# ufukpage/TripleD-Exploring-Depth-Estimation-with-Self-Supervised-Representation-Learning

Hardware: AMD Instinct MI355X
Metric: train imgs/sec at KITTI 192x640 bs=12/GPU (higher is better)
Workload: dtype bf16 convs (MFMA) + f32 loss kernels

## Files before the change

include/tripled_hip.h:

```cpp
#ifndef TRIPLED_HIP_H
#define TRIPLED_HIP_H

#include <stddef.h>
#include <stdint.h>

#ifdef __cplusplus
extern "C" {
#endif

#define TD_ABI_VERSION 3
#define TD_MAX_SRC 4

#define TD_OK 0
#define TD_ERR_BAD_ARG (-1)
#define TD_ERR_UNSUPPORTED (-2)
#define TD_ERR_LAUNCH (-3)
#define TD_ERR_WORKSPACE (-4)

typedef void* td_stream_t;

int td_abi_version(void);
const char* td_error_string(int code);
const char* td_last_hip_error(void);

// ... 90 lines not shown
                     float* workspace, td_stream_t stream);
long long td_conv1x1_wgrad_workspace_floats(long long M, int K, int N);
int td_conv1x1_wgrad(const void* dy, const void* x, long long M, int K, int N, int Hi, int Wi, int stride, int dw_dtype, void* dw,
                     float* workspace, td_stream_t stream);
int td_conv1x1_wgrad_group(int n, const void* const* dy, const void* const* x, const long long* M, const int* K, const int* N,
                           const int* Hi, const int* Wi, const int* stride, const int* dw_dtype, void* const* dw,
                           float* const* workspace, td_stream_t stream);
int td_bn_fwd_from_partials(const void* x, const void* residual, int dtype, const float* gamma, const float* beta,
                            float* running_mean, float* running_var, float momentum, float eps, int relu, long long M,
                            int groups, int C, float* partials, int stat_rows, void* y, float* save_mean,
                            float* save_invstd, td_stream_t stream);

long long td_bias_act_workspace_floats(long long M, int C);
int td_bias_act_fwd(const void* y, const void* bias, int bias_dtype, int dtype, long long M, int C, int act, void* a, td_stream_t stream);
int td_bias_act_bwd(const void* g, const void* a, int dtype, long long M, int C, int act, void* gy, void* dbias, int dbias_dtype,
                    float* workspace, td_stream_t stream);

int td_adam_flat(float* w, const float* grad, float* exp_avg, float* exp_avg_sq, void* lowp, long long n, long long n_lowp,
                 const float* step, const float* lr_dev, float lr_host, double beta1, double beta2, float eps, const float* total_norm,
                 float max_norm, td_stream_t stream);

int td_gather_flat(const void* const* srcs, const long long* dst_offsets, const long long* numels, int n, int src_dtype, float* flat,
                   td_stream_t stream);

int td_bn_partial_rows(long long M, int groups, int C);
int td_bn_fwd_partials(const void* x, int dtype, long long M, int groups, int C, float* partials, td_stream_t stream);
int td_bn_bwd_partials(const void* dy, const void* x, const void* y, int dtype, const float* gamma, const float* beta,
                       const float* save_mean, const float* save_invstd, int relu, long long M, int groups, int C, float* partials,
                       td_stream_t stream);
int td_bn_bwd_from_partials(const void* dy, const void* x, const void* y, int dtype, const float* gamma, const float* beta,
                            const float* save_mean, const float* save_invstd, int relu, long long M, int groups, int C,
                            float* partials, int stat_rows, void* dx, void* dresidual, float* dgamma, float* dbeta,
                            td_stream_t stream);
int td_conv1x1_fwd_bnrelu(const void* z, const void* w, long long M, int groups, int K, int N, float* in_partials, int in_rows,
                          const float* gamma, const float* beta, float* running_mean, float* running_var, float momentum, float eps,
                          float* save_mean, float* save_invstd, void* a_side, void* y, float* stat_partials, td_stream_t stream);
int td_conv1x1_dgrad(const void* dy, const void* w, long long M, int groups, int Cout, int Cin, const void* residual, void* dx,
                     td_stream_t stream);
int td_conv1x1_fwd_sum(const void* x, const void* w, long long M, int K, int N, const void* run_in, void* y, void* run_out,
                       td_stream_t stream);
int td_conv1x1_dgrad_bnsums(const void* dy, const void* w, long long M, int groups, int Cout, int Cin, const void* z,
                            const float* gamma, const float* beta, const float* save_mean, const float* save_invstd, void* dx,
                            float* out_partials, td_stream_t stream);
int td_conv1x1_dgrad_bnbwd(const void* g, const void* z, const void* w, long long M, int groups, int Cout, int Cin, float* in_partials,
                           int in_rows, const float* gamma, const float* beta, const float* save_mean, const float* save_invstd,
                           float* dgamma, float* dbeta, void* dz_side, const void* residual, void* dx, td_stream_t stream);

int td_bn_sync_fwd_sums(const void* x, int dtype, long long M, int groups, int C, float* sums, float* workspace,
                        td_stream_t stream);
int td_bn_sync_fwd_apply(const void* x, const void* residual, int dtype, const float* sums, const float* count,
                         const float* gamma, const float* beta, float* running_mean, float* running_var, float momentum,
                         float eps, int relu, long long M, int groups, int C, void* y, float* save_mean,
                         float* save_invstd, td_stream_t stream);
int td_bn_sync_bwd_sums(const void* dy, const void* x, const void* y, int dtype, const float* gamma, const float* beta,
                        const float* save_mean, const float* save_invstd, int relu, long long M, int groups, int C,
                        float* sums, float* workspace, td_stream_t stream);
int td_bn_sync_bwd_dx(const void* dy, const void* x, const void* y, int dtype, const float* local_sums,
                      const float* global_sums, const float* count, const float* gamma, const float* beta,
                      const float* save_mean, const float* save_invstd, int relu, long long M, int groups, int C,
                      void* dx, void* dresidual, float* dgamma, float* dbeta, float* coef, td_stream_t stream);

int td_edge_weights(const float* img, int B, int h, int w, float a, const float* scale6, float* Wt,
                    td_stream_t stream);
int td_featreg_num_blocks(int B, int h, int w, int C);
int td_featreg_fwd(const void* feat, int dtype, const float* Wt, int B, int h, int w, int C,
                   float* partial, td_stream_t stream);
int td_featreg_bwd(const void* feat, int dtype, const float* Wt, const float* gscale, int B, int h, int w,
                   int C, void* grad, td_stream_t stream);

int td_recon_num_tasks(int B, int h, int w);
int td_recon_fwd(const float* x, const float* y, const float* hole, int B, int h, int w,
                 float* partial, td_stream_t stream);
int td_recon_bwd(const float* x, const float* y, const float* hole, const float* gscale, int B, int h,
                 int w, float* dx, td_stream_t stream);

int td_reflpad1_fwd(const void* in, int dtype, int N, int H, int W, int C, void* out, td_stream_t stream);
int td_reflpad1_bwd(const void* grad_out, int dtype, int N, int H, int W, int C, void* grad_in,
                    td_stream_t stream);

int td_up2_reflpad1_fwd(const void* in, int dtype, int N, int H, int W, int C, void* out, td_stream_t stream);
int td_up2_reflpad1_bwd(const void* grad_out, int dtype, int N, int H, int W, int C, void* grad_in,
                        td_stream_t stream);

int td_featwarp_num_blocks(int B, int h, int w);
int td_featwarp_fwd(const void* tgt, const void* const* src, int n_src, int dtype, const float* disp,
                    const float* P, const float* invK, int B, int h, int w, int C, int hs, int ws,
                    float min_depth, float max_depth, uint8_t* argmin, float* partial, td_stream_t stream);
int td_featwarp_bwd(const void* tgt, const void* const* src, int n_src, int dtype, const float* disp,
                    const float* P, const float* invK, const uint8_t* argmin, const float* gscale,
                    float inv_count, int B, int h, int w, int C, int hs, int ws, float min_depth,
                    float max_depth, void* d_tgt, int* const* d_src, float* d_up, float* dP_partial,
                    td_stream_t stream);
int td_featwarp_dsrc_finish(const int* acc, const float* gscale, float inv_count, int C, long long n, int dtype, void* out,
                            td_stream_t stream);
int td_reduce_partials(const float* partial, int n_src, int B, int blocks_per_sample, float* dP,
                       td_stream_t stream);

int td_l1map_fwd(const void* pred, int dtype, const long long* pred_strides, const float* target, int B, int C,
                 int H, int W, float weight, float* out, td_stream_t stream);
int td_l1map_bwd(const void* pred, int dtype, const long long* pred_strides, const float* target,
                 const float* gmap, int B, int C, int H, int W, float weight, void* dpred, td_stream_t stream);

int td_rgb2lab(const float* rgb, int B, int H, int W, float l_cent, float l_norm, float ab_norm, float* lab,
               td_stream_t stream);

int td_pose_fwd(const float* axisangle, const float* translation, const int* invert, const float* K,
                int n_pairs, int B, float* T, float* P, td_stream_t stream);
int td_pose_bwd(const float* axisangle, const float* translation, const int* invert, const float* K,
                int n_pairs, int B, const float* gT, const float* gP, float* g_axisangle,
                float* g_translation, td_stream_t stream);

int td_color_jitter(const uint8_t* frames_u8, const float* aug, int N, int H, int W, float* means_scratch, float* color,
                    float* color_aug, td_stream_t stream);

int td_fp8_num_blocks(long long n);
int td_fp8_amax_partials(const void* x, int dtype, long long n, float* partials, td_stream_t stream);
int td_fp8_quantize(const void* x, int dtype, long long n, const float* partials, uint8_t* q, float* inv_scale,
                    td_stream_t stream);

#ifdef __cplusplus
}
#endif
#endif
```

tripled-exploring-depth-estimation-with-self-supervised-representation-learning_amd/hostside/mono/model/networks.py:

```python
import os

import numpy as np
import torch
import torch.nn as nn
import torch.nn.functional as F



FUSED_BN_OFF = bool(os.environ.get("TD_NO_FUSED_BN"))


def _ops():
    from tripled_amd import ops
    return ops


def _dense_cl(x):
    if x.is_cuda and x.dim() == 4 and x.shape[1] % 8 == 0 and x.dtype in (torch.float32, torch.bfloat16) \
            and not x.is_contiguous(memory_format=torch.channels_last) and x.stride(1) == 1:
        return x.contiguous(memory_format=torch.channels_last)
    return x


def _fell_back(site, x, why=""):
# ... 451 lines not shown
        self.features = []

    def forward(self, input_image, input_features=None):
        self.features = self.encoder.pyramid(input_image, input_features)
        return self.features

    def stem_only(self, input_image):
        return self.encoder.stem(input_image)


class PoseDecoder(nn.Module):

    def __init__(self, num_ch_enc, stride=1):
        super().__init__()
        self.reduce = Conv2d(int(num_ch_enc[-1]), 256, 1)
        self.conv1 = nn.Conv2d(256, 256, 3, stride, 1)
        self.conv2 = nn.Conv2d(256, 256, 3, stride, 1)
        self.conv3 = nn.Conv2d(256, 6, 1)
        self.relu = nn.ReLU()

    def forward(self, input_features):
        x = self.relu(self.reduce(input_features[-1]))
        x = self.relu(self.conv1(x))
        x = self.relu(self.conv2(x))
        x = self.conv3(x).float()
        x = 0.01 * x.mean(3).mean(2).view(-1, 1, 1, 6)
        return x[..., :3], x[..., 3:]



def upsample(x):
    if x.is_cuda and torch.is_autocast_enabled():
        with torch.autocast("cuda", enabled=False):
            return F.interpolate(x, scale_factor=2, mode="nearest")
    return F.interpolate(x, scale_factor=2, mode="nearest")


class Conv1x1(nn.Module):
    def __init__(self, in_channels, out_channels, bias=False):
        super().__init__()
        self.conv = Conv2d(int(in_channels), int(out_channels), kernel_size=1, stride=1, bias=bias)

    def forward(self, x):
        return self.conv(x)


def _round8(n):
    return (n + 7) // 8 * 8


class _ConvImmediate(torch.autograd.Function):

    @staticmethod
    def forward(ctx, x, w, b):
        with torch.backends.cudnn.flags(enabled=True, benchmark=False):
            y = F.conv2d(x, w, b)
        ctx.save_for_backward(x, w)
        ctx.has_bias = b is not None
        return y

    @staticmethod
    def backward(ctx, gy):
        x, w = ctx.saved_tensors
        with torch.backends.cudnn.flags(enabled=True, benchmark=False):
            gx, gw, gb = torch.ops.aten.convolution_backward(gy, x, w, [w.shape[0]] if ctx.has_bias else None, [1, 1], [0, 0], [1, 1],
                                                              False, [0, 0], 1, [True, True, ctx.has_bias])
        return gx, gw, (gb if ctx.has_bias else None)


class _KeepChannels(torch.autograd.Function):

    @staticmethod
    def forward(ctx, y, c):
        ctx.pad = y.shape[1] - c
        return y.narrow(1, 0, c)

    @staticmethod
    def backward(ctx, g):
        return F.pad(g, (0, 0, 0, 0, 0, ctx.pad)), None


FUSED_BIAS_ACT_OFF = bool(os.environ.get("TD_NO_FUSED_BIAS_ACT"))
FUSED_CRP_OFF = bool(os.environ.get("TD_NO_FUSED_CRP"))


def _activate(y, act):
    if act == "elu":
        return F.elu(y, inplace=True)
    if act == "leaky_relu":
        return F.leaky_relu(y)
    return y


def _conv2d_guarded(x, w, b, act=None):
    if x.is_cuda and x.shape[1] <= 16 and w.shape[0] <= 16 and x.shape[3] > 1024 and torch.backends.cudnn.benchmark:
        if torch.is_autocast_enabled():
            dt = torch.get_autocast_dtype("cuda")
            x, w, b = x.to(dt), w.to(dt), (b.to(dt) if b is not None else None)
        return _activate(_ConvImmediate.apply(x, w, b), act)
    if (act is not None or b is not None) and x.is_cuda and not FUSED_BIAS_ACT_OFF and torch.is_grad_enabled() \
            and torch.is_autocast_enabled() and torch.get_autocast_dtype("cuda") == torch.bfloat16:
        xb = x if x.dtype == torch.bfloat16 else x.to(torch.bfloat16)
        wb = w if w.dtype == torch.bfloat16 else w.to(torch.bfloat16)
        if _ops().conv_bias_act_supported(xb, wb, b, act):
            return _ops().conv_bias_act(xb, wb, b, act)
    return _activate(F.conv2d(x, w, b), act)


class Conv3x3(nn.Module):

    def __init__(self, in_channels, out_channels, use_refl=True):
        super().__init__()
        self.use_refl = use_refl
        self.pad = nn.ReflectionPad2d(1) if use_refl else nn.ZeroPad2d(1)
        self.conv = nn.Conv2d(int(in_channels), int(out_channels), 3)

    def _pad_input(self, x):
        x = _dense_cl(x)
        if self.use_refl and x.shape[1] % 8 == 0 and x.dtype in (torch.float32, torch.bfloat16) \
                and x.is_contiguous(memory_format=torch.channels_last) and x.shape[2] >= 2 and x.shape[3] >= 2:
            from tripled_amd import ops
            return ops.reflpad1(x)
        if self.use_refl:
            _fell_back("Conv3x3.pad", x)
        return self.pad(x)

    def forward(self, x, act=None):
        low_precision = x.is_cuda and (x.dtype == torch.bfloat16 or torch.is_autocast_enabled())
        if not low_precision or os.environ.get("TD_NO_CHANNEL_PAD"):
            return _activate(self.conv(self._pad_input(x) if x.is_cuda else self.pad(x)), act)
        w, b = self.conv.weight, self.conv.bias
        cout, cin = w.shape[0], w.shape[1]
        cin_p, cout_p = _round8(cin), _round8(cout)
        if cin_p == cin and cout_p == cout and x.shape[1] == cin:
            return _conv2d_guarded(self._pad_input(x), w, b, act)
        if x.shape[1] == cin and cin_p != cin:
            x = torch.cat((x, x.new_zeros(x.shape[0], cin_p - cin, x.shape[2], x.shape[3])), 1)
        if x.shape[1] != cin_p:
            raise ValueError("Conv3x3 expects %d (or pre-padded %d) input channels, got %d" % (cin, cin_p, x.shape[1]))
        if not x.is_contiguous(memory_format=torch.channels_last):
            x = x.contiguous(memory_format=torch.channels_last)
        w = F.pad(w, (0, 0, 0, 0, 0, cin_p - cin, 0, cout_p - cout))
        if b is not None and cout_p != cout:
            b = F.pad(b, (0, cout_p - cout))
        if cout_p != cout:
            return _activate(_KeepChannels.apply(_conv2d_guarded(self._pad_input(x), w, b), cout), act)
        return _conv2d_guarded(self._pad_input(x), w, b, act)

    def forward_up(self, x, act=None):
        w, b = self.conv.weight, self.conv.bias
        cout, cin = w.shape[0], w.shape[1]
        x = _dense_cl(x)
        low_precision = x.is_cuda and (x.dtype == torch.bfloat16 or torch.is_autocast_enabled())
        if (self.use_refl and x.is_cuda and x.shape[1] == cin and cin % 8 == 0 and (cout % 8 == 0 or low_precision)
                and x.dtype in (torch.float32, torch.bfloat16) and x.is_contiguous(memory_format=torch.channels_last)
                and not os.environ.get("TD_NO_FUSED_UPSAMPLE")):
            cout_p = _round8(cout)
            if cout_p != cout:
                w = F.pad(w, (0, 0, 0, 0, 0, 0, 0, cout_p - cout))
                b = F.pad(b, (0, cout_p - cout)) if b is not None else None
            if cout_p != cout:
                return _activate(_KeepChannels.apply(_conv2d_guarded(_ops().up2_reflpad1(x), w, b), cout), act)
            return _conv2d_guarded(_ops().up2_reflpad1(x), w, b, act)
        _fell_back("Conv3x3.forward_up", x)
        return self.forward(upsample(x), act)


class Conv5x5(nn.Module):
    def __init__(self, in_channels, out_channels, use_refl=True):
        super().__init__()
        self.pad = nn.ReflectionPad2d(2) if use_refl else nn.ZeroPad2d(2)
        self.conv = nn.Conv2d(int(in_channels), int(out_channels), 5)

    def forward(self, x):
        return self.conv(self.pad(x))


class ConvBlock(nn.Module):
    def __init__(self, in_channels, out_channels):
        super().__init__()
        self.conv = Conv3x3(in_channels, out_channels)
        self.nonlin = nn.ELU(inplace=True)

    def forward(self, x):
        return self.conv(x, act="elu")

    def forward_up(self, x):
        return self.conv.forward_up(x, act="elu")


class CRPBlock(nn.Module):

    def __init__(self, in_planes, out_planes, n_stages):
        super().__init__()
        for i in range(n_stages):
            setattr(self, "{}_{}".format(i + 1, "pointwise"),
                    Conv1x1(in_planes if i == 0 else out_planes, out_planes, False))
        self.stride = 1
        self.n_stages = n_stages
        self.maxpool = nn.MaxPool2d(kernel_size=5, stride=1, padding=2)

    def _pool(self, t):
        if t.is_cuda and t.is_contiguous(memory_format=torch.channels_last) and t.shape[1] % 8 == 0 \
                and t.dtype in (torch.float32, torch.bfloat16):
            from tripled_amd import ops
            return ops.maxpool5(t)
        _fell_back("CRPBlock.maxpool", t)
        return self.maxpool(t)

    def _fused(self, x):
        if FUSED_CRP_OFF or _FP8_1X1[0] or not (self.training and x.is_cuda and torch.is_grad_enabled()):
            return None
        if not (torch.is_autocast_enabled() and torch.get_autocast_dtype("cuda") == torch.bfloat16):
            return None
        convs = [getattr(self, "{}_{}".format(i + 1, "pointwise")).conv for i in range(self.n_stages)]
        if any(c.bias is not None for c in convs):
            return None
        xb = _dense_cl(x if x.dtype == torch.bfloat16 else x.to(torch.bfloat16))
        ws = [c.weight if c.weight.dtype == torch.bfloat16 else c.weight.to(torch.bfloat16) for c in convs]
        if not _ops().crp_supported(xb, ws):
            return None
        return _ops().crp_block(xb, ws)

    def forward(self, x):
        y = self._fused(x)
        if y is not None:
            return y
        top = x
        for i in range(self.n_stages):
            top = getattr(self, "{}_{}".format(i + 1, "pointwise"))(self._pool(top))
            x = top + x
        return x
# ... 37 lines not shown
                setattr(self, "up%d" % i, upshuffle(width, 2))
        self.reduce4 = Conv1x1(num_ch_enc[4], 512, bias=False)
        self.reduce3 = Conv1x1(num_ch_enc[3], width, bias=False)
        self.reduce2 = Conv1x1(num_ch_enc[2], width, bias=False)
        self.reduce1 = Conv1x1(num_ch_enc[1], width, bias=False)
        self.iconv4 = Conv3x3(512, width)
        self.iconv3 = Conv3x3(width * 2 + 1, width)
        self.iconv2 = Conv3x3(width * 2 + 1, width)
        self.iconv1 = Conv3x3(width * 2 + 1, width)
        for i in (4, 3, 2, 1):
            setattr(self, "crp%d" % i, nn.Sequential(CRPBlock(width, width, stages)))
        for i in (4, 3, 2, 1):
            setattr(self, "merge%d" % i, Conv3x3(width, width))
        for i in (4, 3, 2, 1):
            setattr(self, "disp%d" % i, nn.Sequential(Conv3x3(width, 1), nn.Sigmoid()))

    def _stage(self, i, x):
        x = getattr(self, "iconv%d" % i)(x, act="leaky_relu")
        x = getattr(self, "crp%d" % i)(x)
        x = getattr(self, "merge%d" % i)(x, act="leaky_relu")
        head = getattr(self, "disp%d" % i)
        if self.use_shuffle:
            x = getattr(self, "up%d" % (2 if i == 1 else i))(x)
        elif x.is_cuda and x.dtype == torch.bfloat16 and x.is_contiguous(memory_format=torch.channels_last) \
                and x.shape[1] % 8 == 0 and not os.environ.get("TD_NO_FUSED_UPSAMPLE"):
            return x, head[1](head[0].forward_up(x)), True
        else:
            x = upsample(x)
        return x, head(x), False

    def forward(self, input_features, frame_id=0):
        _, l1, l2, l3, l4 = input_features
        l4 = self.do(l4)
        l3 = self.do(l3)
        def joined(r, x, d, deferred):
            if deferred:
                tail = d.to(x.dtype)
                if _ops().join_channels_up2_supported(r, x, tail) and not os.environ.get("TD_NO_CHANNEL_PAD"):
                    return _ops().join_channels_up2(r, x, tail)
                _fell_back("DepthDecoder.join_up2", x)
                x = upsample(x)
            parts = [r, x, d.to(x.dtype)]
            c = sum(p.shape[1] for p in parts)
            if x.is_cuda and c % 8 and x.dtype == torch.bfloat16 and not os.environ.get("TD_NO_CHANNEL_PAD"):
                if _round8(c) == r.shape[1] + x.shape[1] + 8 and _ops().join_channels_supported(*parts):
                    return _ops().join_channels(*parts)
                _fell_back("DepthDecoder.join", x)
                parts.append(x.new_zeros(x.shape[0], _round8(c) - c, x.shape[2], x.shape[3]))
            return torch.cat(parts, 1)

        x, d4, up = self._stage(4, self.reduce4(l4))
        x, d3, up = self._stage(3, joined(self.reduce3(l3), x, d4, up))
        x, d2, up = self._stage(2, joined(self.reduce2(l2), x, d3, up))
        x, d1, up = self._stage(1, joined(self.reduce1(l1), x, d2, up))
        self.outputs = {("disp", frame_id, 3): d4, ("disp", frame_id, 2): d3,
                        ("disp", frame_id, 1): d2, ("disp", frame_id, 0): d1}
        return self.outputs


class Decoder(nn.Module):
    out_key = "res_img"

    def __init__(self, num_ch_enc, num_output_channels=3, num_ch_dec=(16, 32, 64, 128, 256)):
        super().__init__()
        self.num_ch_dec = num_ch_dec
        d = num_ch_dec
        self.upconv5 = ConvBlock(num_ch_enc[4], d[4])
        self.upconv4 = ConvBlock(d[4], d[3])
        self.upconv3 = ConvBlock(d[3], d[2])
        self.upconv2 = ConvBlock(d[2], d[1])
        self.upconv1 = ConvBlock(d[1], d[0])
        self.iconv5 = ConvBlock(d[4], d[4])
        self.iconv4 = ConvBlock(d[3], d[3])
        self.iconv3 = ConvBlock(d[2], d[2])
        self.iconv2 = ConvBlock(d[1], d[1])
        self.iconv1 = ConvBlock(d[0], d[0])
        self.disp4 = Conv3x3(d[3], num_output_channels)
        self.disp3 = Conv3x3(d[2], num_output_channels)
        self.disp2 = Conv3x3(d[1], num_output_channels)
        self.disp1 = Conv3x3(d[0], num_output_channels)
        self.sigmoid = nn.Sigmoid()

    def _heads(self, outputs, key, frame_id, i4, i3, i2, i1):
        outputs[(key, frame_id, 3)] = self.sigmoid(self.disp4(i4))
        outputs[(key, frame_id, 2)] = self.sigmoid(self.disp3(i3))
        outputs[(key, frame_id, 1)] = self.sigmoid(self.disp2(i2))
        outputs[(key, frame_id, 0)] = self.sigmoid(self.disp1(i1))
        return outputs

    def forward(self, input_features, frame_id=0):
        x = self.iconv5.forward_up(self.upconv5(input_features[4]))
        i4 = self.iconv4.forward_up(self.upconv4(x))
        i3 = self.iconv3.forward_up(self.upconv3(i4))
        i2 = self.iconv2.forward_up(self.upconv2(i3))
        i1 = self.iconv1.forward_up(self.upconv1(i2))
        self.outputs = self._heads({}, "res_img", frame_id, i4, i3, i2, i1)
        return self.outputs


class ColorDecoder(Decoder):

    def __init__(self, num_ch_enc, num_output_channels=3, skip_connection_multiplier=1):
        super().__init__(num_ch_enc, num_output_channels, num_ch_dec=(16, 32, 64, 128, 256))
        self.skip_connection_multiplier = skip_connection_multiplier
        d = self.num_ch_dec
        self.upconv5_skip = ConvBlock(num_ch_enc[3], d[3])
        self.upconv4_skip = ConvBlock(num_ch_enc[2], d[2])
        self.upconv3_skip = ConvBlock(num_ch_enc[1], d[1])
        self.upconv2_skip = ConvBlock(num_ch_enc[0], d[0])

    def forward(self, input_features, outputs=None, frame_id=0, skip_layers=(None, None, None, None)):
        e1, e2, e3, e4, e5 = input_features
        m = self.skip_connection_multiplier

        def with_disp(low, scale):
            dsp = F.interpolate(outputs[("disp", frame_id, scale)], [2 * low.shape[2], 2 * low.shape[3]], mode="bilinear",
                                align_corners=False)
            return (dsp * m).to(low.dtype)

        l5 = self.upconv5(e5)
        i5 = self.iconv5.forward_up(l5) + with_disp(l5, 3)
        l4 = self.upconv4(i5)
        if skip_layers[0]:
            l4 = l4 + self.upconv5_skip(e4)
        i4 = self.iconv4.forward_up(l4) + with_disp(l4, 2)
        l3 = self.upconv3(i4)
        if skip_layers[1]:
            l3 = l3 + self.upconv4_skip(e3)
        i3 = self.iconv3.forward_up(l3) + with_disp(l3, 1)
        l2 = self.upconv2(i3)
        if skip_layers[2]:
            l2 = l2 + self.upconv3_skip(e2)
        i2 = self.iconv2.forward_up(l2) + with_disp(l2, 0)
        l1 = self.upconv1(i2)
        if skip_layers[3]:
            l1 = l1 + self.upconv2_skip(e1)
        i1 = self.iconv1.forward_up(l1)
        return self._heads(outputs, "auto_res_img", frame_id, i4, i3, i2, i1)


class IdentityPartial(nn.Module):

    def __init__(self, part_ratio=2, use_right=True):
        super().__init__()
        self.part_ratio = part_ratio
        self.use_right = use_right

    def forward(self, embedding):
        cut = embedding.size(1) // self.part_ratio
        return embedding[:, cut:] if self.use_right else embedding[:, :cut]
```

tripled-exploring-depth-estimation-with-self-supervised-representation-learning_amd/native.py:

```python
import ctypes
import os

import torch

from . import dispatch

_HERE = os.path.dirname(os.path.abspath(__file__))
LIB_PATH = os.path.join(_HERE, "lib", "libtripled_hip.so")

TD_MAX_SRC = 4
_c_float_p = ctypes.c_void_p
_c_u8_p = ctypes.c_void_p

_PTRARR = ctypes.POINTER(ctypes.c_void_p)
_I, _F, _P = ctypes.c_int, ctypes.c_float, ctypes.c_void_p
_LLARR = ctypes.POINTER(ctypes.c_longlong)
_IARR = ctypes.POINTER(ctypes.c_int)
ABI_VERSION = 3

SIGNATURES = {
    "td_abi_version": (_I, []),
    "td_error_string": (ctypes.c_char_p, [_I]),
    "td_last_hip_error": (ctypes.c_char_p, []),
    "td_photo_num_blocks": (_I, [_I, _I, _I]),
    "td_photo_bwd_num_blocks": (_I, [_I, _I, _I]),
    "td_photo_identity": (_I, [_P, _PTRARR, _I, _I, _I, _I, _P, _P, _PTRARR, _P]),
    "td_photo_fwd": (_I, [_P, _PTRARR, _I, _P, _P, _P, _P, _P, _I, _I, _I, _I, _I, _F, _F, _P, _P, _P, _P, _P, _P]),
    "td_photo_bwd": (_I, [_P, _PTRARR, _P, _PTRARR, _I, _P, _P, _P, _P, _P, _I, _P, _F, _I, _I, _I, _I, _I, _F, _F, _P, _P, _P]),
    "td_pack_rgbx": (_I, [_P, _I, _I, _I, _P, _P]),
    "td_upsample_adjoint": (_I, [_P, _I, _I, _I, _I, _I, _P, _I, _P]),
    "td_upsample_adjoint_planes": (_I, [_P, _I, _I, _I, _I, _I, _I, _P, _I, _P]),
    "td_reduce_dP": (_I, [_P, _I, _I, _I, _I, _P, _P]),
    "td_sum_scaled": (_I, [_P, _I, _F, _P, _P]),
    "td_area_downsample": (_I, [_P, _I, _I, _I, _I, _I, _I, _P, _P]),
    "td_smooth_num_blocks": (_I, [_I, _I, _I]),
    "td_smooth_fwd": (_I, [_P, _P, _I, _I, _I, _I, _P, _P, _P]),
    "td_smooth_finish": (_I, [_P, _I, _I, _I, _F, _P, _P]),
    "td_smooth_bwd": (_I, [_P, _P, _P, _I, _I, _I, _I, _P, _F, _P, _P, _P, _I, _P]),
    "td_maxpool5_fwd": (_I, [_P, _I, _I, _I, _I, _I, _P, _P, _P]),
    "td_maxpool5_bwd": (_I, [_P, _P, _I, _I, _I, _I, _I, _P, _P]),
    "td_maxpool5_bwd_add": (_I, [_P, _P, _P, _I, _I, _I, _I, _I, _P, _P]),
    "td_conv1x1_fwd_sum": (_I, [_P, _P, ctypes.c_longlong, _I, _I, _P, _P, _P, _P]),
    "td_maxpool3s2_fwd": (_I, [_P, _I, _I, _I, _I, _I, _P, _P, _P]),
    "td_maxpool3s2_bwd": (_I, [_P, _P, _I, _I, _I, _I, _I, _P, _P]),
    "td_join_fwd": (_I, [_P, _P, _P, _I, ctypes.c_longlong, _I, _I, _I, _P, _P]),
    "td_join_bwd": (_I, [_P, _I, ctypes.c_longlong, _I, _I, _I, _P, _P, _P, _P]),
    "td_join_up2_fwd": (_I, [_P, _P, _P, _I, _I, _I, _I, _I, _I, _I, _P, _P]),
    "td_join_up2_bwd": (_I, [_P, _I, _I, _I, _I, _I, _I, _I, _P, _P, _P, _P]),
    "td_bn_workspace_floats": (ctypes.c_longlong, [ctypes.c_longlong, _I, _I]),
    "td_bn_fwd": (_I, [_P, _P, _I, _P, _P, _P, _P, _F, _F, _I, ctypes.c_longlong, _I, _I, _P, _P, _P, _P, _P]),
    "td_conv1x1_stat_rows": (_I, [ctypes.c_longlong, _I, _I]),
    "td_conv1x1_fwd": (_I, [_P, _P, ctypes.c_longlong, _I, _I, _I, _I, _I, _I, _P, _P, _P]),
    "td_conv3x3_fwd": (_I, [_P, _P, _I, _I, _I, _I, _I, _I, _I, _I, _P, _P, _P]),
    "td_conv3x3_wgrad_workspace_floats": (ctypes.c_longlong, [_I, _I, _I, _I, _I]),
    "td_conv3x3_wgrad": (_I, [_P, _P, _I, _I, _I, _I, _I, _I, _I, _P, _P, _P]),
    "td_conv1x1_wgrad_workspace_floats": (ctypes.c_longlong, [ctypes.c_longlong, _I, _I]),
    "td_conv1x1_wgrad": (_I, [_P, _P, ctypes.c_longlong, _I, _I, _I, _I, _I, _I, _P, _P, _P]),
    "td_conv1x1_wgrad_group": (_I, [_I, _PTRARR, _PTRARR, _LLARR, _IARR, _IARR, _IARR, _IARR, _IARR, _IARR, _PTRARR, _PTRARR, _P]),
    "td_bn_fwd_from_partials": (_I, [_P, _P, _I, _P, _P, _P, _P, _F, _F, _I, ctypes.c_longlong, _I, _I, _P, _I, _P, _P, _P, _P]),
    "td_bias_act_workspace_floats": (ctypes.c_longlong, [ctypes.c_longlong, _I]),
    "td_bias_act_fwd": (_I, [_P, _P, _I, _I, ctypes.c_longlong, _I, _I, _P, _P]),
    "td_bias_act_bwd": (_I, [_P, _P, _I, ctypes.c_longlong, _I, _I, _P, _P, _I, _P, _P]),
    "td_gather_flat": (_I, [_PTRARR, _LLARR, _LLARR, _I, _I, _P, _P]),
    "td_adam_flat": (_I, [_P, _P, _P, _P, _P, ctypes.c_longlong, ctypes.c_longlong, _P, _P, _F, ctypes.c_double, ctypes.c_double, _F, _P, _F, _P]),
    "td_bn_partial_rows": (_I, [ctypes.c_longlong, _I, _I]),
    "td_bn_fwd_partials": (_I, [_P, _I, ctypes.c_longlong, _I, _I, _P, _P]),
    "td_bn_bwd_partials": (_I, [_P, _P, _P, _I, _P, _P, _P, _P, _I, ctypes.c_longlong, _I, _I, _P, _P]),
    "td_bn_bwd_from_partials": (_I, [_P, _P, _P, _I, _P, _P, _P, _P, _I, ctypes.c_longlong, _I, _I, _P, _I, _P, _P, _P, _P, _P]),
    "td_conv1x1_fwd_bnrelu": (_I, [_P, _P, ctypes.c_longlong, _I, _I, _I, _P, _I, _P, _P, _P, _P, _F, _F, _P, _P, _P, _P, _P, _P]),
    "td_conv1x1_dgrad": (_I, [_P, _P, ctypes.c_longlong, _I, _I, _I, _P, _P, _P]),
    "td_conv1x1_dgrad_bnsums": (_I, [_P, _P, ctypes.c_longlong, _I, _I, _I, _P, _P, _P, _P, _P, _P, _P, _P]),
    "td_conv1x1_dgrad_bnbwd": (_I, [_P, _P, _P, ctypes.c_longlong, _I, _I, _I, _P, _I, _P, _P, _P, _P, _P, _P, _P, _P, _P, _P]),
    "td_bn_bwd": (_I, [_P, _P, _P, _I, _P, _P, _P, _P, _I, ctypes.c_longlong, _I, _I, _P, _P, _P, _P, _P, _P]),
    "td_edge_weights": (_I, [_P, _I, _I, _I, _F, ctypes.POINTER(ctypes.c_float), _P, _P]),
    "td_featreg_num_blocks": (_I, [_I, _I, _I, _I]),
    "td_featreg_fwd": (_I, [_P, _I, _P, _I, _I, _I, _I, _P, _P]),
    "td_featreg_bwd": (_I, [_P, _I, _P, _P, _I, _I, _I, _I, _P, _P]),
    "td_recon_num_tasks": (_I, [_I, _I, _I]),
    "td_recon_fwd": (_I, [_P, _P, _P, _I, _I, _I, _P, _P]),
    "td_recon_bwd": (_I, [_P, _P, _P, _P, _I, _I, _I, _P, _P]),
    "td_reflpad1_fwd": (_I, [_P, _I, _I, _I, _I, _I, _P, _P]),
    "td_reflpad1_bwd": (_I, [_P, _I, _I, _I, _I, _I, _P, _P]),
    "td_up2_reflpad1_fwd": (_I, [_P, _I, _I, _I, _I, _I, _P, _P]),
    "td_up2_reflpad1_bwd": (_I, [_P, _I, _I, _I, _I, _I, _P, _P]),
    "td_featwarp_num_blocks": (_I, [_I, _I, _I]),
    "td_featwarp_fwd": (_I, [_P, _PTRARR, _I, _I, _P, _P, _P, _I, _I, _I, _I, _I, _I, _F, _F, _P, _P, _P]),
    "td_featwarp_bwd": (_I, [_P, _PTRARR, _I, _I, _P, _P, _P, _P, _P, _F, _I, _I, _I, _I, _I, _I, _F, _F, _P, _PTRARR,
                             _P, _P, _P]),
    "td_featwarp_dsrc_finish": (_I, [_P, _P, _F, _I, ctypes.c_longlong, _I, _P, _P]),
    "td_reduce_partials": (_I, [_P, _I, _I, _I, _P, _P]),
    "td_bn_sync_fwd_sums": (_I, [_P, _I, ctypes.c_longlong, _I, _I, _P, _P, _P]),
    "td_bn_sync_fwd_apply": (_I, [_P, _P, _I, _P, _P, _P, _P, _P, _P, _F, _F, _I, ctypes.c_longlong, _I, _I, _P, _P, _P, _P]),
    "td_bn_sync_bwd_sums": (_I, [_P, _P, _P, _I, _P, _P, _P, _P, _I, ctypes.c_longlong, _I, _I, _P, _P, _P]),
    "td_bn_sync_bwd_dx": (_I, [_P, _P, _P, _I, _P, _P, _P, _P, _P, _P, _P, _I, ctypes.c_longlong, _I, _I, _P, _P, _P, _P, _P, _P]),
    "td_fp8_num_blocks": (_I, [ctypes.c_longlong]),
    "td_fp8_amax_partials": (_I, [_P, _I, ctypes.c_longlong, _P, _P]),
    "td_fp8_quantize": (_I, [_P, _I, ctypes.c_longlong, _P, _P, _P, _P]),
    "td_color_jitter": (_I, [_P, _P, _I, _I, _I, _P, _P, _P, _P]),
    "td_l1map_fwd": (_I, [_P, _I, _LLARR, _P, _I, _I, _I, _I, _F, _P, _P]),
    "td_l1map_bwd": (_I, [_P, _I, _LLARR, _P, _P, _I, _I, _I, _I, _F, _P, _P]),
    "td_rgb2lab": (_I, [_P, _I, _I, _I, _F, _F, _F, _P, _P]),
    "td_pose_fwd": (_I, [_P, _P, _IARR, _P, _I, _I, _P, _P, _P]),
    "td_pose_bwd": (_I, [_P, _P, _IARR, _P, _I, _I, _P, _P, _P, _P, _P]),
}

DTYPE_CODES = {torch.float32: 0, torch.bfloat16: 1}


class NativeLibraryError(RuntimeError):
    pass


_lib = None


def load(path=None):
    global _lib
    if _lib is not None:
        return _lib
    path = path or os.environ.get("TD_HIP_LIB") or LIB_PATH
    if not os.path.exists(path):
        raise NativeLibraryError(
            "libtripled_hip.so not found at %s -- build it with `python -c 'import __graft_entry__ as g; "
            "g.build()'` or `make -C <package>/csrc`; there is no non-HIP fallback" % path)
    try:
        lib = ctypes.CDLL(path)
    except OSError as e:
        raise NativeLibraryError("cannot load %s: %s" % (path, e)) from e
    for name, (res, args) in SIGNATURES.items():
        try:
            fn = getattr(lib, name)
        except AttributeError as e:
            raise NativeLibraryError("%s does not export %s" % (path, name)) from e
        fn.restype = res
        fn.argtypes = args
    if lib.td_abi_version() != ABI_VERSION:
        raise NativeLibraryError("ABI version mismatch: library %d, binding %d" % (lib.td_abi_version(), ABI_VERSION))
    _lib = lib
    return lib


def check(code, what):
    dispatch.hip(what)
    if code != 0:
        lib = load()
        msg = lib.td_error_string(code).decode()
        hip = lib.td_last_hip_error().decode()
        raise NativeLibraryError("%s failed: %s (%d)%s" % (what, msg, code, (" [" + hip + "]") if hip else ""))


def ptr(t):
    if t is None:
        return None
    if not t.is_cuda:
        raise NativeLibraryError("libtripled_hip needs device tensors (got a %s tensor)" % t.device)
    if not t.is_contiguous():
        raise NativeLibraryError("libtripled_hip needs contiguous tensors")
    return ctypes.c_void_p(t.data_ptr())


def ptr_array(tensors):
    arr = (ctypes.c_void_p * len(tensors))()
    for i, t in enumerate(tensors):
        arr[i] = t.data_ptr()
    return arr


# ... 11 lines not shown
```

tripled-exploring-depth-estimation-with-self-supervised-representation-learning_amd/ops.py:

```python
import os

import torch

from . import native


def _f32c(t):
    if t.dtype != torch.float32:
        t = t.float()
    return t if t.is_contiguous() else t.contiguous()


class PackedFrames:

    def __init__(self, tgt, srcs, pack=True):
        self.tgt_planar = _f32c(tgt.detach())
        self.srcs_planar = tuple(_f32c(s.detach()) for s in srcs)
        if self.tgt_planar.dim() != 4 or self.tgt_planar.shape[1] != 3:
            raise ValueError("colour frames are [B,3,H,W], got %s" % (tuple(self.tgt_planar.shape),))
        B, _, H, W = self.tgt_planar.shape
        self.shape = (B, H, W)
        dev = self.tgt_planar.device
        self.tgt = torch.empty(B, H, W, 4, device=dev, dtype=torch.float32)
        self.srcs = tuple(torch.empty(B, H, W, 4, device=dev, dtype=torch.float32) for _ in self.srcs_planar)
# ... 475 lines not shown
                                   ctx.groups, N, _raw(dyc), _raw(dres) if dres is not None else None, native.ptr(dgamma),
                                   native.ptr(dbeta), native.ptr(ws), native.stream()), "td_bn_bwd")
        if ctx.has_res and not ctx.relu:
            dres = dy
        dx = dw = None
        if ctx.needs_input_grad[0]:
            dx = torch.ops.aten.convolution_backward(dyc, x, w, None, [ctx.stride, ctx.stride], [0, 0], [1, 1], False, [0, 0], 1,
                                                     [True, False, False])[0]
        if ctx.needs_input_grad[1]:
            K, Hi, Wi = x.shape[1], x.shape[2], x.shape[3]
            dw = conv1x1_wgrad(dyc, x, w, M, K, N, Hi, Wi, ctx.stride)
        return dx, dw, dgamma.to(weight.dtype), dbeta.to(weight.dtype), None, None, dres, None, None, None, None, None


def conv1x1_bn_act_supported(x, w, bn_weight, stride=1):
    return (x.is_cuda and x.dim() == 4 and x.dtype == torch.bfloat16 and w.dtype == torch.bfloat16 and w.dim() == 4
            and w.shape[2] == 1 and w.shape[3] == 1 and w.shape[1] == x.shape[1] and x.shape[1] % 64 == 0 and w.shape[0] % 64 == 0
            and stride in (1, 2) and bn_weight is not None and bn_weight.dtype == torch.float32
            and x.is_contiguous(memory_format=torch.channels_last)
            and (w.is_contiguous() or w.is_contiguous(memory_format=torch.channels_last)))


def conv1x1_bn_act(x, w, weight, bias, running_mean, running_var, momentum, eps, residual=None, relu=False, groups=1, stride=1):
    if x.shape[0] % groups:
        raise ValueError("batch %d is not %d stacked passes" % (x.shape[0], groups))
    if not conv1x1_bn_act_supported(x, w, weight, stride):
        raise native.NativeLibraryError("conv1x1_bn_act needs bf16 channels_last HIP tensors with Cin % 64 == Cout % 64 == 0")
    if residual is not None and (residual.dtype != x.dtype or not residual.is_contiguous(memory_format=torch.channels_last)):
        residual = residual.to(x.dtype).contiguous(memory_format=torch.channels_last)
    return _Conv1x1BatchNormAct.apply(x, w, weight, bias, running_mean, running_var, residual, momentum, eps, relu, groups, stride)


ACT_CODES = {None: 0, "elu": 1, "leaky_relu": 2}


class _ConvBiasAct(torch.autograd.Function):

    @staticmethod
    def forward(ctx, x, w, b, act):
        lib = native.load()
        y = torch.ops.aten.convolution(x, w, None, [1, 1], [0, 0], [1, 1], False, [0, 0], 1)
        if not y.is_contiguous(memory_format=torch.channels_last):
            y = y.contiguous(memory_format=torch.channels_last)
        B, C, H, W = y.shape
        native.check(lib.td_bias_act_fwd(_raw(y), _raw(b) if b is not None else None, native.DTYPE_CODES[b.dtype] if b is not None else 0,
                                         native.DTYPE_CODES[y.dtype], B * H * W, C, ACT_CODES[act], _raw(y), native.stream()),
                     "td_bias_act_fwd")
        ctx.save_for_backward(x, w, y if act is not None else None, b)
        ctx.act = act
        return y

    @staticmethod
    def backward(ctx, g):
        lib = native.load()
        x, w, a, b = ctx.saved_tensors
        B, C, H, W = g.shape
        if g.dtype != w.dtype or not g.is_contiguous(memory_format=torch.channels_last):
            g = g.to(w.dtype).contiguous(memory_format=torch.channels_last)
        M = B * H * W
        gy = torch.empty_like(g, memory_format=torch.channels_last) if ctx.act is not None else g
        db = torch.empty_like(b) if b is not None and ctx.needs_input_grad[2] else None
        ws = torch.empty(lib.td_bias_act_workspace_floats(M, C), device=g.device, dtype=torch.float32)
        if ctx.act is not None or db is not None:
            native.check(lib.td_bias_act_bwd(_raw(g), _raw(a) if a is not None else None, native.DTYPE_CODES[g.dtype], M, C,
                                             ACT_CODES[ctx.act], _raw(gy) if ctx.act is not None else None,
                                             _raw(db) if db is not None else None, native.DTYPE_CODES[db.dtype] if db is not None else 0,
                                             native.ptr(ws), native.stream()), "td_bias_act_bwd")
        dx, dw, _ = torch.ops.aten.convolution_backward(gy, x, w, None, [1, 1], [0, 0], [1, 1], False, [0, 0], 1,
                                                        [ctx.needs_input_grad[0], ctx.needs_input_grad[1], False])
        return dx, dw, db, None


def conv_bias_act_supported(x, w, b, act):
    cout = w.shape[0]
    return (act in ACT_CODES and x.is_cuda and x.dim() == 4 and x.dtype == torch.bfloat16 and w.dtype == torch.bfloat16
            and x.is_contiguous(memory_format=torch.channels_last) and (b is None or b.dtype in native.DTYPE_CODES)
            and 8 <= cout <= 256 and cout % 8 == 0 and 256 % (cout // 8) == 0 and x.shape[1] == w.shape[1])


def conv_bias_act(x, w, b, act=None):
    if not conv_bias_act_supported(x, w, b, act):
        raise native.NativeLibraryError("conv_bias_act needs bf16 channels_last HIP tensors, Cout in {8, 16, 32, 64, 128, 256}")
    return _ConvBiasAct.apply(x, w, b, act)


_WGRAD_QUEUE = None
WGRAD_GROUP = os.environ.get("TD_WGRAD_GROUP", "node")


class wgrad_group:

    def __init__(self, assign=False, scope="node"):
        self.assign, self.scope, self.items = assign, scope, []

    def __enter__(self):
        global _WGRAD_QUEUE
        self.prev = _WGRAD_QUEUE
        self.active = WGRAD_GROUP == self.scope and not (self.prev is not None and self.prev.assign)
        if self.active:
            _WGRAD_QUEUE = self
        return self

    def __exit__(self, *exc):
        global _WGRAD_QUEUE
        if self.active:
            _WGRAD_QUEUE = self.prev
            if self.items and exc[0] is None:
                flush_wgrads(self.items)
        return False


def deferred_wgrads():
    return wgrad_group(assign=True, scope="step")


def flush_wgrads(queue):
    import ctypes
    lib = native.load()
    n = len(queue)
    P, LL, I = (ctypes.c_void_p * n), (ctypes.c_longlong * n), (ctypes.c_int * n)
    dy, x, dw, ws = P(), P(), P(), P()
    for i, q in enumerate(queue):
        dy[i], x[i], dw[i], ws[i] = q["dy"].data_ptr(), q["x"].data_ptr(), q["dw"].data_ptr(), q["ws"].data_ptr()
    native.check(lib.td_conv1x1_wgrad_group(n, dy, x, LL(*[q["M"] for q in queue]), I(*[q["K"] for q in queue]),
                                            I(*[q["N"] for q in queue]), I(*[q["Hi"] for q in queue]), I(*[q["Wi"] for q in queue]),
                                            I(*[q["stride"] for q in queue]), I(*[native.DTYPE_CODES[q["dw"].dtype] for q in queue]),
                                            dw, ws, native.stream()), "td_conv1x1_wgrad_group")
    for q in queue:
        w = q["w"]
        if w is None:
            continue
        if w.grad is None:
            w.grad = q["dw"]
        else:
            w.grad.add_(q["dw"])


def conv1x1_wgrad(dz, inp, w, M, K, N, Hi, Wi, stride):
    lib = native.load()
    dw = torch.empty_like(w)
    wsw = torch.empty(lib.td_conv1x1_wgrad_workspace_floats(M, K, N), device=dz.device, dtype=torch.float32)
    q = _WGRAD_QUEUE
    if q is not None and (not q.assign or (w.is_leaf and w.requires_grad)):
        q.items.append(dict(dy=dz, x=inp, dw=dw, ws=wsw, w=w if q.assign else None, M=M, K=K, N=N, Hi=Hi, Wi=Wi, stride=stride))
        return None if q.assign else dw
    native.check(lib.td_conv1x1_wgrad(_raw(dz), _raw(inp), M, K, N, Hi, Wi, stride, native.DTYPE_CODES[w.dtype], _raw(dw),
                                      native.ptr(wsw), native.stream()), "td_conv1x1_wgrad")
    return dw


def conv3x3_wgrad_wins(B, Ho, Wo, C, N, stride):
    return stride == 1 and C == 64 and N == 64 and Wo >= 160 and Ho >= 48 and B * Ho * Wo < (1 << 31) - 128


def conv3x3_wgrad(dy, x, w, pad):
    lib = native.load()
    B, N, Ho, Wo = dy.shape
    C = x.shape[1]
    dw = torch.empty_like(w, memory_format=torch.channels_last)
    ws = torch.empty(lib.td_conv3x3_wgrad_workspace_floats(B, Ho, Wo, C, N), device=x.device, dtype=torch.float32)
    native.check(lib.td_conv3x3_wgrad(_raw(dy), _raw(x), B, Ho, Wo, C, N, pad, native.DTYPE_CODES[w.dtype], _raw(dw), native.ptr(ws),
                                      native.stream()), "td_conv3x3_wgrad")
    return dw


class BnState:
# ... 656 lines not shown
```

Before: 439.9.

## Add fused reflect-pad/upsample 3x3 narrow-channel conv kernel with bias, activation, sigmoid

Adds a custom MFMA HIP kernel for 3x3 convolutions with few output channels (8-32) that builds the reflection-padded, optionally 2x-upsampled input patch in shared memory and applies bias and activation, including sigmoid for the disparity heads. The goal is to avoid separate pad/upsample, conv, bias/act and sigmoid kernels and the intermediate tensors they write for high-resolution decoder layers. A shape allowlist limits it to specific decoder layer shapes. Backward still goes through explicit padding and the library convolution_backward, with extra sigmoid_backward and padding steps.

```diff
diff --git a/include/tripled_hip.h b/include/tripled_hip.h
--- a/include/tripled_hip.h
+++ b/include/tripled_hip.h
@@ -196,6 +196,9 @@
 int td_up2_reflpad1_bwd(const void* grad_out, int dtype, int N, int H, int W, int C, void* grad_in,
                         td_stream_t stream);
 
+int td_conv3x3_narrow_fwd(const void* x, const void* w, const void* bias, int bias_dtype, int B, int H, int W, int Cin, int N,
+                          int up2, int act, int n_store, void* y, td_stream_t stream);
+
 int td_featwarp_num_blocks(int B, int h, int w);
 int td_featwarp_fwd(const void* tgt, const void* const* src, int n_src, int dtype, const float* disp,
                     const float* P, const float* invK, int B, int h, int w, int C, int hs, int ws,
diff --git a/tripled-exploring-depth-estimation-with-self-supervised-representation-learning_amd/csrc/td_conv3x3_narrow.hip b/tripled-exploring-depth-estimation-with-self-supervised-representation-learning_amd/csrc/td_conv3x3_narrow.hip
--- /dev/null
+++ b/tripled-exploring-depth-estimation-with-self-supervised-representation-learning_amd/csrc/td_conv3x3_narrow.hip
@@ -0,0 +1,148 @@
+#include <hip/hip_bf16.h>
+
+#include "td_common.h"
+#include "td_conv_tile.h"
+#include "td_vec8.h"
+
+namespace td {
+
+constexpr int NC_TH = 8, NC_TW = 32;
+constexpr int NC_PH = NC_TH + 2, NC_PW = NC_TW + 2;
+
+__device__ __forceinline__ float nc_act(float z, int act) {
+  if (act == 1) return z > 0.f ? z : expm1f(z);
+  if (act == 2) return z > 0.f ? z : 0.01f * z;
+  if (act == 3) return 1.f / (1.f + expf(-bf2f(f2bf(z))));
+  return z;
+}
+
+template <int CIN, bool UP2>
+__global__ __launch_bounds__(CV_THREADS) void conv3x3_narrow_fwd_kernel(const __hip_bfloat16* __restrict__ x, const __hip_bfloat16* __restrict__ w,
+                                                                        const void* __restrict__ bias, int bias_bf16, int H, int W, int N,
+                                                                        int tiles_x, int tiles_y, int act, int n_store,
+                                                                        __hip_bfloat16* __restrict__ y) {
+  constexpr int PITCH = CIN * 2 + 16, KS = CIN / 16, CX = CIN / 8;
+  __shared__ __attribute__((aligned(16))) unsigned char patch[NC_PH * NC_PW * PITCH];
+  const int tid = threadIdx.x, lane = tid & 63, wv = tid >> 6, l31 = lane & 31, h = lane >> 5;
+  int t = blockIdx.x;
+  const int tx = t % tiles_x;
+  t /= tiles_x;
+  const int ty = t % tiles_y, b = t / tiles_y;
+  const int r0 = ty * NC_TH, c0 = tx * NC_TW;
+  const int Hs = UP2 ? H >> 1 : H, Ws = UP2 ? W >> 1 : W;
+
+  const __hip_bfloat16* xb = x + (size_t)b * Hs * Ws * CIN;
+  constexpr int NCH = NC_PH * NC_PW * CX, ITERS = (NCH + CV_THREADS - 1) / CV_THREADS;
+#pragma unroll
+  for (int it = 0; it < ITERS; ++it) {
+    const int i = tid + it * CV_THREADS;
+    if (i < NCH) {
+      const int p = i / CX, cv = i - p * CX;
+      const int py = p / NC_PW, px = p - py * NC_PW;
+      int sy = reflect1(r0 + py - 1, H), sx = reflect1(c0 + px - 1, W);
+      if (UP2) { sy >>= 1; sx >>= 1; }
+      const uint4 v = *reinterpret_cast<const uint4*>(xb + ((size_t)sy * Ws + sx) * CIN + cv * 8);
+      *reinterpret_cast<uint4*>(patch + p * PITCH + cv * 16) = v;
+    }
+  }
+
+  cv_bf16x8 wf[9][KS];
+#pragma unroll
+  for (int tap = 0; tap < 9; ++tap)
+#pragma unroll
+    for (int ks = 0; ks < KS; ++ks) {
+      uint4 v = make_uint4(0u, 0u, 0u, 0u);
+      if (l31 < N) v = *reinterpret_cast<const uint4*>(w + ((size_t)l31 * 9 + tap) * CIN + ks * 16 + h * 8);
+      wf[tap][ks] = __builtin_bit_cast(cv_bf16x8, v);
+    }
+  float bv[16];
+#pragma unroll
+  for (int g = 0; g < 4; ++g)
+#pragma unroll
+    for (int r = 0; r < 4; ++r) {
+      const int c = 8 * g + 4 * h + r;
+      bv[4 * g + r] = (!bias || c >= N) ? 0.f
+                      : bias_bf16  ? bf2f(reinterpret_cast<const unsigned short*>(bias)[c])
+                                   : reinterpret_cast<const float*>(bias)[c];
+    }
+  __syncthreads();
+
+  cv_f32x16 acc[2];
+#pragma unroll
+  for (int j = 0; j < 2; ++j)
+#pragma unroll
+    for (int e = 0; e < 16; ++e) acc[j][e] = 0.f;
+#pragma unroll
+  for (int ky = 0; ky < 3; ++ky)
+#pragma unroll
+    for (int kx = 0; kx < 3; ++kx)
+#pragma unroll
+      for (int ks = 0; ks < KS; ++ks)
+#pragma unroll
+        for (int j = 0; j < 2; ++j) {
+          const int p = (2 * wv + j + ky) * NC_PW + l31 + kx;
+          const cv_bf16x8 fx = __builtin_bit_cast(cv_bf16x8, *reinterpret_cast<const uint4*>(patch + p * PITCH + ks * 32 + h * 16));
+          acc[j] = __builtin_amdgcn_mfma_f32_32x32x16_bf16(wf[ky * 3 + kx][ks], fx, acc[j], 0, 0, 0);
+        }
+
+#pragma unroll
+  for (int j = 0; j < 2; ++j) {
+    const int row = r0 + 2 * wv + j, col = c0 + l31;
+    const bool valid = row < H && col < W;
+    const size_t pix = ((size_t)b * H + row) * W + col;
+    uint2 pk[4];
+#pragma unroll
+    for (int g = 0; g < 4; ++g) {
+      unsigned short o[4];
+#pragma unroll
+      for (int r = 0; r < 4; ++r) o[r] = f2bf(nc_act(bf2f(f2bf(acc[j][4 * g + r])) + bv[4 * g + r], act));
+      pk[g].x = (unsigned)o[0] | ((unsigned)o[1] << 16);
+      pk[g].y = (unsigned)o[2] | ((unsigned)o[3] << 16);
+    }
+    if (n_store > 0) {
+      if (valid && h == 0) {
+        unsigned short* yp = reinterpret_cast<unsigned short*>(y) + pix * n_store;
+        const unsigned short o[4] = {(unsigned short)(pk[0].x & 0xffff), (unsigned short)(pk[0].x >> 16),
+                                     (unsigned short)(pk[0].y & 0xffff), (unsigned short)(pk[0].y >> 16)};
+#pragma unroll
+        for (int r = 0; r < 4; ++r)
+          if (r < n_store) yp[r] = o[r];
+      }
+      continue;
+    }
+#pragma unroll
+    for (int gp = 0; gp < 2; ++gp) {
+      const uint2 mine = h ? pk[2 * gp + 1] : pk[2 * gp], send = h ? pk[2 * gp] : pk[2 * gp + 1];
+      uint2 recv;
+      recv.x = (unsigned)__shfl_xor((int)send.x, 32, 64);
+      recv.y = (unsigned)__shfl_xor((int)send.y, 32, 64);
+      const uint4 out = h ? make_uint4(recv.x, recv.y, mine.x, mine.y) : make_uint4(mine.x, mine.y, recv.x, recv.y);
+      const int c = 16 * gp + 8 * h;
+      if (valid && c < N) *reinterpret_cast<uint4*>(y + pix * N + c) = out;
+    }
+  }
+}
+
+}
+
+extern "C" int td_conv3x3_narrow_fwd(const void* x, const void* w, const void* bias, int bias_dtype, int B, int H, int W, int Cin, int N,
+                                     int up2, int act, int n_store, void* y, td_stream_t stream) {
+  if (!x || !w || !y || B <= 0 || H <= 0 || W <= 0) return TD_ERR_BAD_ARG;
+  if ((Cin != 16 && Cin != 32 && Cin != 64) || N < 8 || N > 32 || N % 8 != 0 || H < 2 || W < 2 || act < 0 || act > 3 || n_store < 0 ||
+      n_store > 4 || (up2 && ((H | W) & 1)) || (bias && bias_dtype != TD_DTYPE_BF16 && bias_dtype != TD_DTYPE_F32))
+    return TD_ERR_UNSUPPORTED;
+  const int tiles_x = (W + td::NC_TW - 1) / td::NC_TW, tiles_y = (H + td::NC_TH - 1) / td::NC_TH;
+  const long long blocks = (long long)B * tiles_x * tiles_y;
+  if (blocks >= (1ll << 31) || (long long)B * H * W * 64 >= (1ll << 40)) return TD_ERR_UNSUPPORTED;
+  hipStream_t st = (hipStream_t)stream;
+  const int bb = bias_dtype == TD_DTYPE_BF16;
+#define TD_NC_F(CIN, UP)                                                                                                       \
+  hipLaunchKernelGGL((td::conv3x3_narrow_fwd_kernel<CIN, UP>), dim3((unsigned)blocks), dim3(td::CV_THREADS), 0, st,             \
+                     (const __hip_bfloat16*)x, (const __hip_bfloat16*)w, bias, bb, H, W, N, tiles_x, tiles_y, act, n_store,     \
+                     (__hip_bfloat16*)y)
+  if (Cin == 16) { if (up2) TD_NC_F(16, true); else TD_NC_F(16, false); }
+  else if (Cin == 32) { if (up2) TD_NC_F(32, true); else TD_NC_F(32, false); }
+  else { if (up2) TD_NC_F(64, true); else TD_NC_F(64, false); }
+#undef TD_NC_F
+  return td::record_launch_error(hipGetLastError(), "td_conv3x3_narrow_fwd");
+}
diff --git a/tripled-exploring-depth-estimation-with-self-supervised-representation-learning_amd/hostside/mono/model/networks.py b/tripled-exploring-depth-estimation-with-self-supervised-representation-learning_amd/hostside/mono/model/networks.py
--- a/tripled-exploring-depth-estimation-with-self-supervised-representation-learning_amd/hostside/mono/model/networks.py
+++ b/tripled-exploring-depth-estimation-with-self-supervised-representation-learning_amd/hostside/mono/model/networks.py
@@ -557,6 +557,7 @@
 
 FUSED_BIAS_ACT_OFF = bool(os.environ.get("TD_NO_FUSED_BIAS_ACT"))
 FUSED_CRP_OFF = bool(os.environ.get("TD_NO_FUSED_CRP"))
+NARROW_CONV_OFF = bool(os.environ.get("TD_NO_NARROW_CONV"))
 
 
 def _activate(y, act):
@@ -564,6 +565,8 @@
         return F.elu(y, inplace=True)
     if act == "leaky_relu":
         return F.leaky_relu(y)
+    if act == "sigmoid":
+        return torch.sigmoid(y)
     return y
 
 
@@ -600,7 +603,36 @@
             _fell_back("Conv3x3.pad", x)
         return self.pad(x)
 
+    def _narrow(self, x, act, up2):
+        w, b = self.conv.weight, self.conv.bias
+        cout, cin = w.shape[0], w.shape[1]
+        if NARROW_CONV_OFF or not (self.use_refl and x.is_cuda and x.dim() == 4 and x.shape[1] == cin and cin in (16, 32, 64)
+                                   and _round8(cout) <= 32 and torch.is_grad_enabled() and torch.is_autocast_enabled()
+                                   and torch.get_autocast_dtype("cuda") == torch.bfloat16):
+            return None
+        m = 2 if up2 else 1
+        if not _ops().conv3x3_narrow_wins(m * x.shape[2], m * x.shape[3], cin, _round8(cout), up2, "fwd"):
+            return None
+        cout_p = _round8(cout)
+        keep = cout if cout_p != cout else None
+        if keep is None and act == "sigmoid" or keep is not None and (keep > 4 or act not in (None, "sigmoid")):
+            return None
+        x = _dense_cl(x)
+        xb = x if x.dtype == torch.bfloat16 else x.to(torch.bfloat16)
+        wb = w if w.dtype == torch.bfloat16 else w.to(torch.bfloat16)
+        if keep is not None:
+            wb = F.pad(wb, (0, 0, 0, 0, 0, 0, 0, cout_p - cout))
+            b = F.pad(b, (0, cout_p - cout)) if b is not None else None
+        if not _ops().conv3x3_narrow_supported(xb, wb, b, act, up2, keep):
+            return None
+        return _ops().conv3x3_narrow(xb, wb, b, act, up2, keep)
+
     def forward(self, x, act=None):
+        y = self._narrow(x, act, False)
+        if y is not None:
+            return y
+        if act == "sigmoid":
+            return torch.sigmoid(self.forward(x))
         low_precision = x.is_cuda and (x.dtype == torch.bfloat16 or torch.is_autocast_enabled())
         if not low_precision or os.environ.get("TD_NO_CHANNEL_PAD"):
             return _activate(self.conv(self._pad_input(x) if x.is_cuda else self.pad(x)), act)
@@ -623,6 +655,9 @@
         return _conv2d_guarded(self._pad_input(x), w, b, act)
 
     def forward_up(self, x, act=None):
+        y = self._narrow(x, act, True)
+        if y is not None:
+            return y
         w, b = self.conv.weight, self.conv.bias
         cout, cin = w.shape[0], w.shape[1]
         x = _dense_cl(x)
@@ -826,10 +861,10 @@
         self.sigmoid = nn.Sigmoid()
 
     def _heads(self, outputs, key, frame_id, i4, i3, i2, i1):
-        outputs[(key, frame_id, 3)] = self.sigmoid(self.disp4(i4))
-        outputs[(key, frame_id, 2)] = self.sigmoid(self.disp3(i3))
-        outputs[(key, frame_id, 1)] = self.sigmoid(self.disp2(i2))
-        outputs[(key, frame_id, 0)] = self.sigmoid(self.disp1(i1))
+        outputs[(key, frame_id, 3)] = self.disp4(i4, act="sigmoid")
+        outputs[(key, frame_id, 2)] = self.disp3(i3, act="sigmoid")
+        outputs[(key, frame_id, 1)] = self.disp2(i2, act="sigmoid")
+        outputs[(key, frame_id, 0)] = self.disp1(i1, act="sigmoid")
         return outputs
 
     def forward(self, input_features, frame_id=0):
diff --git a/tripled-exploring-depth-estimation-with-self-supervised-representation-learning_amd/native.py b/tripled-exploring-depth-estimation-with-self-supervised-representation-learning_amd/native.py
--- a/tripled-exploring-depth-estimation-with-self-supervised-representation-learning_amd/native.py
+++ b/tripled-exploring-depth-estimation-with-self-supervised-representation-learning_amd/native.py
@@ -83,6 +83,7 @@
     "td_reflpad1_bwd": (_I, [_P, _I, _I, _I, _I, _I, _P, _P]),
     "td_up2_reflpad1_fwd": (_I, [_P, _I, _I, _I, _I, _I, _P, _P]),
     "td_up2_reflpad1_bwd": (_I, [_P, _I, _I, _I, _I, _I, _P, _P]),
+    "td_conv3x3_narrow_fwd": (_I, [_P, _P, _P, _I, _I, _I, _I, _I, _I, _I, _I, _I, _P, _P]),
     "td_featwarp_num_blocks": (_I, [_I, _I, _I]),
     "td_featwarp_fwd": (_I, [_P, _PTRARR, _I, _I, _P, _P, _P, _I, _I, _I, _I, _I, _I, _F, _F, _P, _P, _P]),
     "td_featwarp_bwd": (_I, [_P, _PTRARR, _I, _I, _P, _P, _P, _P, _P, _F, _I, _I, _I, _I, _I, _I, _F, _F, _P, _PTRARR,
diff --git a/tripled-exploring-depth-estimation-with-self-supervised-representation-learning_amd/ops.py b/tripled-exploring-depth-estimation-with-self-supervised-representation-learning_amd/ops.py
--- a/tripled-exploring-depth-estimation-with-self-supervised-representation-learning_amd/ops.py
+++ b/tripled-exploring-depth-estimation-with-self-supervised-representation-learning_amd/ops.py
@@ -581,6 +581,92 @@
     if not conv_bias_act_supported(x, w, b, act):
         raise native.NativeLibraryError("conv_bias_act needs bf16 channels_last HIP tensors, Cout in {8, 16, 32, 64, 128, 256}")
     return _ConvBiasAct.apply(x, w, b, act)
+
+
+NARROW_ACT_CODES = {None: 0, "elu": 1, "leaky_relu": 2, "sigmoid": 3}
+
+
+class _Conv3x3Narrow(torch.autograd.Function):
+
+    @staticmethod
+    def forward(ctx, x, w, b, act, up2, keep):
+        lib = native.load()
+        B, C, Hs, Ws = x.shape
+        H, W = (2 * Hs, 2 * Ws) if up2 else (Hs, Ws)
+        N = w.shape[0]
+        wc = w if w.is_contiguous(memory_format=torch.channels_last) else w.contiguous(memory_format=torch.channels_last)
+        y = torch.empty((B, keep or N, H, W), device=x.device, dtype=x.dtype, memory_format=torch.channels_last)
+        native.check(lib.td_conv3x3_narrow_fwd(_raw(x), _raw(wc), _raw(b) if b is not None else None,
+                                               native.DTYPE_CODES[b.dtype] if b is not None else 0, B, H, W, C, N, int(up2),
+                                               NARROW_ACT_CODES[act], int(keep or 0), _raw(y), native.stream()), "td_conv3x3_narrow_fwd")
+        ctx.save_for_backward(x, w, y if act is not None else None, b)
+        ctx.act, ctx.up2, ctx.keep = act, up2, keep
+        return y
+
+    @staticmethod
+    def backward(ctx, g):
+        lib = native.load()
+        x, w, a, b = ctx.saved_tensors
+        N = w.shape[0]
+        act = ctx.act
+        if g.dtype != w.dtype:
+            g = g.to(w.dtype)
+        if act == "sigmoid":
+            g, act, a = torch.ops.aten.sigmoid_backward(g, a), None, None
+        if ctx.keep:
+            g = torch.nn.functional.pad(g, (0, 0, 0, 0, 0, N - ctx.keep))
+        if not g.is_contiguous(memory_format=torch.channels_last):
+            g = g.contiguous(memory_format=torch.channels_last)
+        B, _, H, W = g.shape
+        M = B * H * W
+        gy = torch.empty_like(g, memory_format=torch.channels_last) if act is not None else g
+        db = torch.empty_like(b) if b is not None and ctx.needs_input_grad[2] else None
+        if act is not None or db is not None:
+            ws = torch.empty(lib.td_bias_act_workspace_floats(M, N), device=g.device, dtype=torch.float32)
+            native.check(lib.td_bias_act_bwd(_raw(g), _raw(a) if a is not None else None, native.DTYPE_CODES[g.dtype], M, N,
+                                             ACT_CODES[act], _raw(gy) if act is not None else None,
+                                             _raw(db) if db is not None else None, native.DTYPE_CODES[db.dtype] if db is not None else 0,
+                                             native.ptr(ws), native.stream()), "td_bias_act_bwd")
+        C, Hs, Ws = x.shape[1], x.shape[2], x.shape[3]
+        pad_fwd, pad_bwd, what = (lib.td_up2_reflpad1_fwd, lib.td_up2_reflpad1_bwd, "td_up2_reflpad1") if ctx.up2 else \
+            (lib.td_reflpad1_fwd, lib.td_reflpad1_bwd, "td_reflpad1")
+        xp = torch.empty((B, C, H + 2, W + 2), device=x.device, dtype=x.dtype, memory_format=torch.channels_last)
+        native.check(pad_fwd(_raw(x), native.DTYPE_CODES[x.dtype], B, Hs, Ws, C, _raw(xp), native.stream()), what + "_fwd")
+        dxp, dw, _ = torch.ops.aten.convolution_backward(gy, xp, w, None, [1, 1], [0, 0], [1, 1], False, [0, 0], 1,
+                                                         [ctx.needs_input_grad[0], ctx.needs_input_grad[1], False])
+        dx = None
+        if dxp is not None:
+            if not dxp.is_contiguous(memory_format=torch.channels_last):
+                dxp = dxp.contiguous(memory_format=torch.channels_last)
+            dx = torch.empty_like(x, memory_format=torch.channels_last)
+            native.check(pad_bwd(_raw(dxp), native.DTYPE_CODES[dxp.dtype], B, Hs, Ws, C, _raw(dx), native.stream()), what + "_bwd")
+        return dx, dw, db, None, None, None
+
+
+CONV3X3_NARROW_FWD_WINS = frozenset({
+    (48, 160, 64, 32, False), (48, 160, 64, 32, True), (48, 160, 64, 8, False), (48, 160, 64, 8, True),
+    (96, 320, 32, 32, False), (96, 320, 32, 32, True), (96, 320, 32, 16, False), (96, 320, 32, 16, True),
+    (96, 320, 32, 8, False), (96, 320, 32, 8, True),
+    (192, 640, 16, 16, False), (192, 640, 16, 16, True), (192, 640, 16, 8, False), (192, 640, 16, 8, True)})
+
+
+def conv3x3_narrow_wins(Ho, Wo, Cin, N, up2, direction="fwd"):
+    return direction == "fwd" and (Ho, Wo, Cin, N, bool(up2)) in CONV3X3_NARROW_FWD_WINS
+
+
+def conv3x3_narrow_supported(x, w, b, act, up2=False, keep=None):
+    N = w.shape[0]
+    return (act in NARROW_ACT_CODES and x.is_cuda and x.dim() == 4 and x.dtype == torch.bfloat16 and w.dtype == torch.bfloat16
+            and x.is_contiguous(memory_format=torch.channels_last) and x.shape[1] in (16, 32, 64) and x.shape[1] == w.shape[1]
+            and tuple(w.shape[2:]) == (3, 3) and N in (8, 16, 32) and x.shape[2] >= (1 if up2 else 2)
+            and x.shape[3] >= (1 if up2 else 2) and (b is None or (b.dtype in native.DTYPE_CODES and b.numel() == N))
+            and (keep is None or (1 <= keep <= 4 and keep < N and act in (None, "sigmoid"))) and (act != "sigmoid" or keep is not None))
+
+
+def conv3x3_narrow(x, w, b, act=None, up2=False, keep=None):
+    if not conv3x3_narrow_supported(x, w, b, act, up2, keep):
+        raise native.NativeLibraryError("conv3x3_narrow needs bf16 channels_last HIP tensors, Cin in {16, 32, 64}, Cout in {8, 16, 32}")
+    return _Conv3x3Narrow.apply(x, w, b, act, bool(up2), keep)
 
 
 _WGRAD_QUEUE = None
```

New measurement: 439.3. Within noise of the previous version (-0.2%).
